# albertz/ParseOggVorbis

Measured on AMD Instinct MI355X. Metric: audio packets/sec (blocksize 2048, stereo), higher is better.
Workload: dtype f32; 1 GPU; config3: 65536 stereo packets, blocksize 2048, 64 streams x 1024, floor+coupling+IMDCT+window+overlap-add; packets_per_gpu=65536, parallelism=streams sharded over 1 GPU(s), no data-path collective

## Files before the change

### parseoggvorbis_amd/csrc/vorbis_synth_hip.hip

```cpp
#include <hip/hip_runtime.h>

#include <mutex>
#include <string>

#include <stdlib.h>

#include "vsyn_host.h"
#include "vsyn_device.h"
#include "vsyn_staged.h"
#include "vsyn_prep.h"
#include "vsyn_fused.h"
#include "vsyn_fused_u.h"
#include "vsyn_vq.h"
#include "vsyn_pcm.h"
#include "vsyn_features.h"
#include "vsyn_spectral.h"
#include "vsyn_spectral_lin.h"
#include "vsyn_chroma.h"
#include "vsyn_spectral_post.h"
#include "vsyn_pcen.h"
#include "vsyn_hpss.h"
#include "vsyn_istft.h"
#include "vsyn_effects.h"
#include "vsyn_pv.h"
// ... 664 lines not shown
  }
  if (!force_staged) {
    FusedArgs a;
    a.cb = h->d_const;
    a.binseg = h->fused.d_binseg;
    a.lds_image = h->fused.d_lds;
    a.packets = d_packets;
    a.segs = d_segments;
    a.info = info;
    a.sinfo = sinfo;
    a.run_cls = h->ws_runcls[wb].p;
    a.runs_per_seg = runs_per_seg;
    a.residue = d_residue;
    a.curve = taps ? taps->floor_curve : nullptr;
    a.fy = fy;
    a.pcm = d_pcm;
    a.carry = h->d_carry;
    a.status = h->d_status;
    a.plane_stride = plane_stride;
    a.S = S;
    a.R = R;
    a.fused_ok = use_u ? (fmask & 1u) : fmask;
    a.coupling_mode = (uint32_t)h->fused.coupling_mode;
    if (staged_may_work) HIPCHK(hipEventRecord(h->ev_join, h->side));
    const bool time_u = use_u && (h->profile_which == 2 || !(fmask & 1u));
    hipError_t e = hipSuccess;
    if (a.fused_ok) {
      if (!time_u && (h->profile_which == 1 || h->profile_which == 2)) HIPCHK(profile_begin(h, s, a.curve ? "vsyn_fused_tap_kernel" : fused_kernel_name(H)));
      e = fused_launch(H, h->fused, a, s);
      if (e != hipSuccess) return fail(err, VSYN_ERR_HIP, "fused launch failed: %s", hipGetErrorString(e));
      if (!time_u && (h->profile_which == 1 || h->profile_which == 2)) HIPCHK(profile_end(h, s));
    }
    if (use_u) {
      FusedArgs au = a;
      au.fused_ok = fmask;
      if (time_u && (h->profile_which == 1 || h->profile_which == 2)) HIPCHK(profile_begin(h, s, au.curve ? "vsyn_fused_u_tap_kernel" : "vsyn_fused_u_kernel"));
      e = u_launch(H, h->utab, au, s);
      if (e != hipSuccess) return fail(err, VSYN_ERR_HIP, "generic fused launch failed: %s", hipGetErrorString(e));
      if (time_u && (h->profile_which == 1 || h->profile_which == 2)) HIPCHK(profile_end(h, s));
    }
    if (staged_may_work) HIPCHK(hipStreamWaitEvent(s, h->ev_join, 0));
  }

  h->last_ran_layout = !prep_kernel;
  h->last_prep_on_main = ps == s;
  h->pre_done_valid[wb] = ps != s;
// ... 1990 lines not shown
```

### parseoggvorbis_amd/csrc/vsyn_fused.h

```cpp
#pragma once
#include <hip/hip_runtime.h>

#include "vsyn_device.h"

#ifndef FUSED_WAVES
#define FUSED_WAVES 16
#endif
#ifndef FUSED_MIN_WAVES_PER_SIMD
#define FUSED_MIN_WAVES_PER_SIMD 4
#endif
#define FUSED_XSLOTS 576
#ifndef VSYN_KNOCKOUT
#define VSYN_KNOCKOUT 0
#endif
#ifdef VSYN_STAMPS
#define VSYN_NSTAMPS 16
__device__ unsigned long long g_vsyn_stamps[8192][VSYN_NSTAMPS];
#define STAMP(i)                                                  \
  do {                                                            \
    __builtin_amdgcn_sched_barrier(0);                            \
    const unsigned long long t_ = __builtin_readcyclecounter();   \
    st_acc[i] += t_ - st_last;                                    \
    st_last = t_;                                                 \
    __builtin_amdgcn_sched_barrier(0);                            \
  } while (0)
#else
#define STAMP(i) do { } while (0)
#endif

struct FusedLdsImage {
  float2 pre[8][64];
  float2 post[8][64];
  float2 tw1[8][64];
  float2 tw2[8][8];
  float win[2][2][8][64];
  float invdb[260];
  float2 pre_s[64];
  float2 post_s[64];
  float2 tws[6][64];
  float wsl[2][64];
  float2 post8[8][8];
  float wsl8[2][8][8];
};

struct FusedTables {
  uint8_t* d_binseg = nullptr;
  FusedLdsImage* d_lds = nullptr;
  int waves_per_cu = 12;
  int coupling_mode = 0;
};

struct FusedArgs {
  const uint8_t* cb;
  const uint8_t* binseg;
  const FusedLdsImage* lds_image;
  const vsyn_packet* packets;
  const vsyn_segment* segs;
  const PktInfo* info;
  const SegInfo* sinfo;
  uint16_t* curve;
  const uint8_t* run_cls;
  const float* residue;
  const uint16_t* fy;
  float* pcm;
  float* carry;
  DevStatus* status;
  uint64_t plane_stride;
  uint32_t S, R, fused_ok, coupling_mode, runs_per_seg;
};

__device__ __forceinline__ float2 f2(float x, float y) { return make_float2(x, y); }
__device__ __forceinline__ float2 cadd(float2 a, float2 b) { return f2(a.x + b.x, a.y + b.y); }
__device__ __forceinline__ float2 csub(float2 a, float2 b) { return f2(a.x - b.x, a.y - b.y); }
__device__ __forceinline__ float2 cmulf(float2 a, float2 b) {
  return f2(__builtin_fmaf(a.x, b.x, -(a.y * b.y)), __builtin_fmaf(a.x, b.y, a.y * b.x));
}
__device__ __forceinline__ float2 mul_mi(float2 a) { return f2(a.y, -a.x); }

__device__ __forceinline__ void dft8(float2 (&x)[8]) {
  const float h = 0.70710678118654752440f;
  float2 a0 = cadd(x[0], x[4]), a1 = cadd(x[1], x[5]), a2 = cadd(x[2], x[6]), a3 = cadd(x[3], x[7]);
  float2 b0 = csub(x[0], x[4]), b1 = csub(x[1], x[5]), b2 = csub(x[2], x[6]), b3 = csub(x[3], x[7]);
  b1 = f2((b1.x + b1.y) * h, (b1.y - b1.x) * h);
  b2 = mul_mi(b2);
  b3 = f2((b3.y - b3.x) * h, -(b3.x + b3.y) * h);
  float2 c0 = cadd(a0, a2), c1 = csub(a0, a2), c2 = cadd(a1, a3), c3 = mul_mi(csub(a1, a3));
  x[0] = cadd(c0, c2);
  x[4] = csub(c0, c2);
  x[2] = cadd(c1, c3);
  x[6] = csub(c1, c3);
  float2 d0 = cadd(b0, b2), d1 = csub(b0, b2), d2 = cadd(b1, b3), d3 = mul_mi(csub(b1, b3));
// ... 98 lines not shown
  k.bad = (r[7] >> 8) & 0xFFu;
  return k;
}
__device__ __forceinline__ PktScalars pkt_load(const PktInfo* p) {
  typedef const __attribute__((address_space(4))) u32x8* const_words;
  return pkt_fields(*(const_words)(uintptr_t)p);
}

enum { K_REG = 0, K_LDS = 1, K_CARRY = 2 };
__device__ __forceinline__ uint32_t bitrev6(uint32_t l) { return __brev(l) >> 26; }

template <int ROLE, bool TAPC>
__device__ __forceinline__ uint32_t fused_short_pass(const FusedArgs& A, const FusedLdsImage& T, float2* __restrict__ xb, const float2* __restrict__ pxb,
                                                     float2* seg2, lds_f32* cbuf, lds_u32* my_flags, const lds_u32* partner_flags, const uint32_t lane,
                                                     const vsyn_segment sg, const SegInfo si, const uint32_t q, const uint32_t qa, const uint32_t qb,
                                                     const uint32_t C, const uint32_t c, float* plane, const PktInfo* ip, const uint32_t epoch,
                                                     const uint32_t prev_kind, const uint32_t prev_half, float (&P)[8], const uint32_t bseg0,
                                                     const uint32_t sidx, const uint32_t xsl, const uint32_t posts, const uint32_t ys_stride, bool& hand_over_out
#ifdef VSYN_STAMPS
                                                     , unsigned long long (&st_acc)[VSYN_NSTAMPS], unsigned long long& st_last
#endif
                                                     ) {
  constexpr uint32_t MS = 128u, ML = 1024u;
  const ConstHeader* H = hdr_of(A.cb);
  typedef uint32_t u32x4 __attribute__((ext_vector_type(4)));
  const uint32_t idx = min(q + (lane & 7u), qb - 1u);
  const u32x4 da = ((const u32x4*)(ip + idx))[0], db = ((const u32x4*)(ip + idx))[1];
  const uint32_t map0 = __builtin_amdgcn_readfirstlane(db[3] & 0xFFu);
  const bool cand = lane < 8u && q + lane < qb;
  const uint64_t okm = __ballot(cand && !((db[3] >> 8) & 0xFFu) && !((db[2] >> 16) & 0xFFu) && (db[3] & 0xFFu) == map0);
  const uint32_t Jp = (uint32_t)__builtin_ctzll(~okm);
  STAMP(9);
  const uint32_t qn = q + Jp, p0 = sg.first_packet + q;
  const uint32_t emit_l = q + (lane & 7u) < qa ? 0u : da[3];
  float2 raw[8];
  uint32_t vrow[8];
#pragma unroll
  for (uint32_t t = 0; t < 8; ++t) {
    const uint32_t tc = min(t, Jp - 1u);
    const uint64_t off = ((uint64_t)__builtin_amdgcn_readlane(da[1], tc) << 32) | (uint32_t)__builtin_amdgcn_readlane(da[0], tc);
    raw[t] = (VSYN_KNOCKOUT & 256) ? f2(0.001f * (float)lane, 0.002f) : ((const float2*)(A.residue + off + (size_t)c * MS))[lane];
    vrow[t] = (A.fy + ((size_t)(p0 + tc) * C + c) * ys_stride)[sidx];
  }
#pragma unroll
  for (uint32_t t = 0; t < 8; ++t)
    if (t >= Jp) raw[t] = f2(0.f, 0.f);
  float2 r[8];
// ... 171 lines not shown
        float* up = out + shift + 2u * kap;
        float* dn = out + shift + MS - 2u - 2u * kap;
#pragma unroll
        for (int j = 0; j < 4; ++j) {
          *(float2*)(up + 16 * j) = f2(oh_s[j], n_s[j]);
          *(float2*)(dn - 16 * j) = f2(n_m[j], oh_m[j]);
        }
      }
    } else if (emit) {
#pragma unroll
      for (int j = 0; j < 4; ++j) {
        const uint32_t s = 2u * kap + 16u * j;
        const uint32_t f0 = s + shift, f1 = s + 1u + shift, f2m = MS - 2u - s + shift, f3m = MS - 1u - s + shift;
        if (f0 < emit) out[f0] = oh_s[j];
        if (f1 < emit) out[f1] = n_s[j];
        if (f2m < emit) out[f2m] = n_m[j];
        if (f3m < emit) out[f3m] = oh_m[j];
      }
    }
  }
  (void)next_emit;
  (void)next_out;
  if ((last_of_segment || hand_over) && jo == Jp - 1u) {
    const size_t carry_half = (size_t)H->max_streams * C * ML;
    float* cout = A.carry + (si.parity_in ^ 1u) * carry_half + ((size_t)sg.stream * C + c) * ML;
#pragma unroll
    for (int k = 0; k < 8; ++k) {
      const uint32_t f = kap + 8u * k;
      const uint32_t s = k >= 4 ? 2u * f - 64u : 63u - 2u * f, sm = MS - 1u - s;
      const float v_s = Pn[k] * wl1[k], v_m = Pn[k] * wl0[k];
      if (last_of_segment) {
        cout[s] = v_s;
        cout[sm] = v_m;
      } else {
        cbuf[s] = v_s;
        cbuf[sm] = v_m;
      }
    }
  }
  {
    const int from = (int)((Jp - 1u) * 8u + kap);
#pragma unroll
    for (int k = 0; k < 8; ++k) P[k] = __shfl(Pn[k], from);
  }
  if (__any(floor_bad)) {
    if (floor_bad) raise_status(A.status, VSYN_ST_FLOOR_VALUE, floor_bad_pkt);
    vmem_drain();
  }
  hand_over_out = hand_over;
  return Jp;
}


template <int ROLE, bool MIXED, bool TAPC, bool RING = false>
__device__ __forceinline__ void fused_run(const FusedArgs& A, const FusedLdsImage& T, float2* __restrict__ xb, const float2* __restrict__ pxb, float4* __restrict__ seg,
                                          lds_f32* cbuf, lds_u32* my_flags, const lds_u32* partner_flags, const uint32_t lane0, const uint32_t g,
                                          const vsyn_segment sg, const SegInfo si, const uint32_t qa, const uint32_t qb, const uint32_t C, const uint32_t c,
                                          const RingLds& rl = RingLds()) {
  static_assert(!(RING && MIXED), "ring mode is a steady-run mode");
  constexpr uint32_t STEP = RING ? 8u : 1u;
  constexpr uint32_t ML = 1024;
  const uint8_t* __restrict__ cb = A.cb;
  const ConstHeader* H = hdr_of(cb);
  const uint32_t num = sg.num_packets;

  float P[8];
#pragma unroll
  for (int k = 0; k < 8; ++k) P[k] = 0.f;
  uint32_t prev_next_long = 1;
  uint32_t prev_kind = K_REG;
  uint32_t prev_half = 0;
  float* const plane = A.pcm + ((size_t)g * C + c) * A.plane_stride;
  const float* cin = nullptr;

  const uint32_t seg_base = (uint32_t)(uintptr_t)(lds_u32*)seg;
  uint32_t bseg[8];
#pragma unroll
  for (int t = 0; t < 8; ++t) bseg[t] = seg_base | (seg_base << 16);
  uint32_t sidx = 0, xsl = 0;
  int cur_floor = -1;
  uint32_t vrow = 0;
  bool vrow_ok = false;

  const uint32_t ys_stride = __builtin_amdgcn_readfirstlane(H->ys_stride);
  const MapConst* const maps = (const MapConst*)(cb + H->off_map);
  const FloorConst* const floors = (const FloorConst*)(cb + H->off_floor);
  uint32_t cur_map = 0xFFFFFFFFu, map_floor = 0, posts = 0;

  const uint32_t q0 = RING ? ((rl.slot == 7u && qa) ? qa - 1u : qa + rl.slot) : (qa ? qa - 1 : 0);
  if (RING && q0 >= qb) return;
  bool ring_dead = false;
  const PktInfo* const ip = A.info + __builtin_amdgcn_readfirstlane(sg.first_packet);
  PktScalars pi = pkt_load(ip + q0);
  float2 raw[8];
  bool raw_ahead = false;
  bool dma_ahead = false;
  uint32_t dma_younger = 0;
  auto issue_dma = [&](uint64_t off, const uint32_t ln) {
    const char* gsrc = (const char*)(A.residue + off) + 16u * ln;
#pragma unroll
    for (int i = 0; i < 4; ++i)
      __builtin_amdgcn_global_load_lds((const __attribute__((address_space(1))) void*)(gsrc + 1024 * i),
                                       (__attribute__((address_space(3))) void*)((lds_u32*)xb + 256 * i), 16, 0, 0);
  };
  if (!MIXED) {
    const float2* src = (const float2*)(A.residue + pi.res_off + (size_t)c * ML) + lane0;
#pragma unroll
    for (int t = 0; t < 8; ++t) raw[t] = stream_load2(src + 64 * t);
  }
  if (MIXED && qa == 0 && si.has_carry && !pi.bad) {
    const size_t carry_half = (size_t)H->max_streams * C * ML;
    cin = A.carry + si.parity_in * carry_half + ((size_t)sg.stream * C + c) * ML;
    const bool carry_long = si.carry_n == 2u * ML;
    prev_half = si.carry_n / 2u;
    if (carry_long && pi.lng) {
      prev_kind = K_CARRY;
    } else {
      const uint32_t base = carry_long ? 448u : 0u;
      if (carry_long)
        for (uint32_t i = lane0; i < min(448u, pi.emit); i += 64) plane[pi.out_pos + i] = cin[i];
      cbuf[lane0] = cin[base + lane0];
      cbuf[lane0 + 64u] = cin[base + lane0 + 64u];
      prev_kind = K_LDS;
    }
  }
  uint32_t lane_v = lane0;
  vmem_drain();
#ifdef VSYN_STAMPS
  unsigned long long st_acc[VSYN_NSTAMPS] = {0, 0, 0, 0, 0, 0, 0, 0, 0, 0, 0, 0, 0, 0, 0, 0};
  unsigned long long st_last = __builtin_readcyclecounter();
#endif
  uint32_t q = q0;
  for (uint32_t it = 0; q < qb; ++it, q += STEP) {
    STAMP(0);
    asm volatile("" : "+v"(lane_v));
    const uint32_t lane = lane_v;
    const uint32_t kappa = ((lane & 7u) << 3) | (lane >> 3);
    const uint32_t p = sg.first_packet + q;
    const bool halo = q < qa, has_next = q + STEP < qb;
    const PktScalars pin = pkt_load(ip + (has_next ? q + STEP : q));
    if (RING) prev_next_long = q ? (pkt_load(ip + q - 1u).widx >> 1) & 1u : 1u;
    const bool lng = !MIXED || pi.lng != 0u;
    const bool nlng = !MIXED || pin.lng != 0u;
    const uint32_t M = lng ? ML : 128u;
    if (MIXED && pi.bad) {
#pragma unroll
      for (int k = 0; k < 8; ++k) P[k] = 0.f;
      prev_kind = K_REG;
      prev_half = 0;
      vrow_ok = false;
      pi = pin;
      continue;
    }
    if (pi.mapping != cur_map) {
      cur_map = pi.mapping;
      {
        typedef const __attribute__((address_space(4))) uint32_t* kptr;
        const uint32_t w = *(kptr)(uintptr_t)((const uint8_t*)maps[cur_map].chfloor + (c & ~3u));
        map_floor = (w >> (8u * (c & 3u))) & 0xFFu;
      }
    }
    if (MIXED && !lng) {
      if (cur_floor != (int)map_floor) {
        const FloorConst* fc = floors + map_floor;
        posts = __builtin_amdgcn_readfirstlane(fc->posts);
        const uint8_t* bs = A.binseg + (size_t)map_floor * ML;
        const uint32_t seg_base0 = (uint32_t)(uintptr_t)(lds_u32*)seg;
#pragma unroll
        for (int t = 0; t < 8; ++t) {
          const uint32_t two = *(const uint16_t*)(bs + 2u * (lane + 64u * t));
          bseg[t] = (seg_base0 + 8u * (two & 0xFFu)) | ((seg_base0 + 8u * (two >> 8)) << 16);
        }
        const bool in = lane < posts;
        sidx = in ? fc->sorted_idx[lane] : 0u;
        xsl = in ? fc->xs_sorted[lane] : 0u;
        cur_floor = (int)map_floor;
        vmem_drain();
      }
      bool ho = false;
      const uint32_t Jp = fused_short_pass<ROLE, TAPC>(A, T, xb, pxb, (float2*)seg, cbuf, my_flags, partner_flags, lane, sg, si, q, qa, qb, C, c, plane, ip, it + 1u,
                                                 prev_kind, prev_half, P, bseg[0], sidx, xsl, posts, ys_stride, ho
#ifdef VSYN_STAMPS
                                                 , st_acc, st_last
#endif
                                                 );
      prev_kind = ho ? K_LDS : K_REG;
      prev_half = 128u;
      prev_next_long = 0u;
      vrow_ok = false;
      q += Jp - 1u;
      pi = pkt_load(ip + min(q + 1u, qb - 1u));
      STAMP(8);
      continue;
    }

    float2 r[8];
    auto residue_rows = [&](const bool L) {
      if (MIXED && L) {
        if (!dma_ahead) {
          issue_dma(pi.res_off + (uint64_t)c * ML, lane);
          dma_younger = 0;
        }
        if (dma_younger == 8u) __builtin_amdgcn_s_waitcnt(0x0F78);
        else vmem_drain();
        dma_ahead = false;
        if (ROLE != 0) {
          pair_post(&my_flags[0], it + 1);
          pair_wait(&partner_flags[0], it + 1);
        }
#pragma unroll
        for (int t = 0; t < 8; ++t) {
          const float2 own = xb[t * 64 + lane];
          if (ROLE == 0) {
            r[t] = own;
          } else {
// ... 30 lines not shown
    };
    if (lng) residue_rows(true);
    else residue_rows(false);
    STAMP(1);
    if (ROLE != 0 && !(VSYN_KNOCKOUT & 1)) pair_post(&my_flags[1], it + 1);
    if (!MIXED) {
      const float2* src = (const float2*)(A.residue + pin.res_off + (size_t)c * ML) + lane;
#pragma unroll
      for (int t = 0; t < 8; ++t) raw[t] = stream_load2(src + 64 * t);
    }
    __builtin_amdgcn_sched_barrier(0);

    bool floor_bad = false;
    float2* const seg2 = (float2*)seg;
    if (VSYN_KNOCKOUT & 16) {
      if (it == 0) seg2[lane] = f2(0.f, 200.5f);
    } else if (!((pi.own >> c) & 1u)) {
      seg2[lane] = f2(0.f, ((pi.used >> c) & 1u) ? 256.5f : 255.5f);
    } else {
      const uint32_t f = map_floor;
      const uint16_t* row = A.fy + ((size_t)p * C + c) * ys_stride;
      uint32_t v = vrow;
      if (cur_floor != (int)f) {
        const FloorConst* fc = floors + f;
        posts = __builtin_amdgcn_readfirstlane(fc->posts);
        const uint8_t* bs = A.binseg + (size_t)f * ML;
#pragma unroll
        for (int t = 0; t < 8; ++t) {
          const uint32_t two = *(const uint16_t*)(bs + 2u * (lane + 64u * t));
          bseg[t] = (seg_base + 8u * (two & 0xFFu)) | ((seg_base + 8u * (two >> 8)) << 16);
        }
        const bool in = lane < posts;
        sidx = in ? fc->sorted_idx[lane] : 0u;
        xsl = in ? fc->xs_sorted[lane] : 0u;
        cur_floor = (int)f;
        v = row[sidx];
        vmem_drain();
      } else if (!vrow_ok) {
        v = row[sidx];
        vmem_drain();
      }
      if (lane >= posts) v = 0;
      const uint64_t mask = __ballot((v >> 15) != 0) | 1ull;
      const uint64_t below = mask & ((2ull << lane) - 1ull);
      const uint32_t lo = 63u - (uint32_t)__clzll((long long)below);
      const uint64_t above = lane < 63u ? (mask >> (lane + 1u)) : 0ull;
      const bool has_hi = above != 0ull;
      const uint32_t hi = lane + (uint32_t)__ffsll((long long)above);
      const uint32_t packed = (xsl << 16) | (v & 0x7FFFu);
      const uint32_t plo = (uint32_t)__shfl((int)packed, (int)lo);
      const uint32_t phi = (uint32_t)__shfl((int)packed, (int)(has_hi ? hi : lo));
      floor_bad = (v & 0x7FFFu) > 255u;
      const float x0 = (float)(plo >> 16), y0 = fminf((float)(plo & 0xFFFFu), 255.f);
      const float x1 = (float)(phi >> 16), y1 = fminf((float)(phi & 0xFFFFu), 255.f);
      const float inv = has_hi ? __builtin_amdgcn_rcpf(x1 - x0) : 0.f;
      const float ady = fabsf(y1 - y0);
      const float a = ady * inv, b = __builtin_fmaf(-ady, x0, 0.5f) * inv;
      seg2[lane] = y1 >= y0 ? f2(a, b + y0) : f2(-a, (y0 + 1.f) - b);
// ... 160 lines not shown
#pragma unroll
        for (int j = 0; j < 4; ++j) {
          if (!MIXED) {
            stream_store2(up + 128 * j, oh_s[j], n_s[j]);
            stream_store2(dn - 128 * j, n_m[j], oh_m[j]);
          } else {
            *(float2*)(up + 128 * j) = f2(oh_s[j], n_s[j]);
            *(float2*)(dn - 128 * j) = f2(n_m[j], oh_m[j]);
          }
        }
      } else if (emit) {
        if (MIXED) dma_younger = 0xFFu;
#pragma unroll
        for (int j = 0; j < 4; ++j) {
          const uint32_t s = 2u * kappa + 128u * j;
          const uint32_t f0 = s + shift, f1 = s + 1u + shift, f2m = 1022u - s + shift, f3m = 1023u - s + shift;
          if (f0 < emit) out[f0] = oh_s[j];
          if (f1 < emit) out[f1] = n_s[j];
          if (f2m < emit) out[f2m] = n_m[j];
          if (f3m < emit) out[f3m] = oh_m[j];
        }
      }
      STAMP(8);
      if (MIXED && (last_of_segment || hand_over)) dma_younger = 0xFFu;
      if (last_of_segment || hand_over) {
        const size_t carry_half = (size_t)H->max_streams * C * ML;
        float* cout = A.carry + (si.parity_in ^ 1u) * carry_half + ((size_t)sg.stream * C + c) * ML;
        float* nxt = plane + pin.out_pos;
        const float (*TN)[8][64] = T.win[cur_next_long];
#pragma unroll
        for (int k = 0; k < 8; ++k) {
          const uint32_t m = kappa + 64u * k;
          const uint32_t s = k >= 4 ? 2u * m - 512u : 511u - 2u * m;
          const float v_s = P[k] * TN[1][k][lane], v_m = P[k] * TN[0][k][lane];
          if (last_of_segment) {
            cout[s] = v_s;
            cout[1023u - s] = v_m;
          } else {
            const uint32_t sm = 1023u - s;
            if (s < 448u) {
              if (s < pin.emit) nxt[s] = v_s;
            } else if (s < 576u) {
              cbuf[s - 448u] = v_s;
            }
            if (sm < 448u) {
              if (sm < pin.emit) nxt[sm] = v_m;
            } else if (sm < 576u) {
              cbuf[sm - 448u] = v_m;
            }
          }
        }
        if (!MIXED) vmem_drain();
      }
    } else {
    }
    if (MIXED) {
      prev_kind = hand_over ? K_LDS : K_REG;
      prev_half = M;
    }
    if (__any(floor_bad)) {
      if (lane == 0) raise_status(A.status, VSYN_ST_FLOOR_VALUE, p);
      vmem_drain();
    }
    prev_next_long = cur_next_long;
    pi = pin;
  }
#ifdef VSYN_STAMPS
  if (lane0 == 0) {
    const uint32_t unit = blockIdx.x * FUSED_WAVES + (threadIdx.x >> 6);
    if (unit < 8192)
      for (int i = 0; i < VSYN_NSTAMPS; ++i) g_vsyn_stamps[unit][i] = i == VSYN_NSTAMPS - 1 ? (unsigned long long)(qb - q0) : st_acc[i];
  }
#endif
}

static_assert(FUSED_WAVES % 2 == 0, "the two channel waves of a run must share a workgroup");
template <bool TAPC>
__device__ __forceinline__ void fused_kernel_body(const FusedArgs& A) {
  struct Lds {
    float4 seg[FUSED_WAVES][64];
    uint32_t flag[FUSED_WAVES][4];
    FusedLdsImage t;
    float2 x[FUSED_WAVES][FUSED_XSLOTS];
    float ring[FUSED_WAVES][8 * 64];
  };
  __shared__ Lds s_lds;
  FusedLdsImage& s_t = s_lds.t;
  float2 (&s_x)[FUSED_WAVES][FUSED_XSLOTS] = s_lds.x;
  float4 (&s_seg)[FUSED_WAVES][64] = s_lds.seg;
  uint32_t (&s_flag)[FUSED_WAVES][4] = s_lds.flag;
  static_assert(sizeof(s_lds.seg) + sizeof(s_lds.flag) < 65536, "floor entry addresses are packed into 16 bits");
  const ConstHeader* H = hdr_of(A.cb);
  const uint32_t wave = __builtin_amdgcn_readfirstlane(threadIdx.x >> 6);
  const uint32_t lane = threadIdx.x & 63u;
  const uint32_t C = H->channels;
  const uint32_t per_seg = A.runs_per_seg * C;
  const uint32_t unit = blockIdx.x * FUSED_WAVES + wave;
  const uint32_t g = __builtin_amdgcn_readfirstlane(unit / per_seg);
  const uint32_t rem = unit - g * per_seg;
  const uint32_t run = __builtin_amdgcn_readfirstlane(rem / C), c = __builtin_amdgcn_readfirstlane(rem % C);
  vsyn_segment sg = {};
  SegInfo si = {};
  uint32_t cls = 0xFFu;
  bool seg_ok = false;
  if (g < A.S) {
    sg = A.segs[g];
    if (sg.stream < H->max_streams && !(sg.residue_off & 3)) {
      seg_ok = true;
      si = A.sinfo[g];
      cls = __builtin_amdgcn_readfirstlane((uint32_t)A.run_cls[(size_t)g * A.runs_per_seg + run]);
    }
  }
  const uint32_t qa = run * A.R;
  const uint32_t qb = min(sg.num_packets, qa + A.R);
  const bool active = (cls == 1u && (A.fused_ok & 1u)) || (cls == 2u && (A.fused_ok & 2u));
  if (!__syncthreads_or(active ? 1 : 0)) return;
  {
    const uint4* src = (const uint4*)A.lds_image;
    uint4* dst = (uint4*)&s_t;
    for (uint32_t i = threadIdx.x; i < sizeof(FusedLdsImage) / 16; i += FUSED_WAVES * 64) dst[i] = src[i];
    if (threadIdx.x < FUSED_WAVES * 4) (&s_flag[0][0])[threadIdx.x] = 0u;
  }
  static_assert(FUSED_WAVES == 16, "ring mode: 8 slots x 2 channels");
  const uint32_t unit0 = blockIdx.x * FUSED_WAVES;
  const bool one_seg = unit0 / per_seg == (unit0 + FUSED_WAVES - 1u) / per_seg;
  const bool ring_ok = C == 2u && one_seg && g < A.S && (A.fused_ok & 1u) && seg_ok && (cls == 1u || qa >= sg.num_packets);
  const bool ring = __syncthreads_and(ring_ok ? 1 : 0);
  if (!ring && !active) return;
  const uint32_t mag = A.coupling_mode == 1 ? 0u : 1u;
  const int role = (A.coupling_mode == 0 || C < 2) ? 0 : (c == mag ? 1 : 2);
  const uint32_t pw = role ? (wave ^ 1u) : wave;
  lds_u32* mf = (lds_u32*)s_flag[wave];
  const lds_u32* pf = (const lds_u32*)s_flag[pw];
  lds_f32* cbw = (lds_f32*)((float*)s_seg[wave] + 128);
  if (ring) {
    const uint32_t slot = wave >> 1, pred = ((slot + 7u) & 7u) * 2u + c, succ = ((slot + 1u) & 7u) * 2u + c;
    RingLds rl;
    rl.mine = (lds_f32*)s_lds.ring[wave];
    rl.pred = (const lds_f32*)s_lds.ring[pred];
    rl.flags = (lds_u32*)&s_flag[wave][2];
    rl.pred_flags = (const lds_u32*)&s_flag[pred][2];
    rl.succ_flags = (const lds_u32*)&s_flag[succ][2];
    rl.slot = slot;
    const uint32_t ca = qa - slot * A.R, ce = min(sg.num_packets, ca + 8u * A.R);
    if (role == 0) fused_run<0, false, TAPC, true>(A, s_t, s_x[wave], s_x[pw], s_seg[wave], cbw, mf, pf, lane, g, sg, si, ca, ce, C, c, rl);
    else if (role == 1) fused_run<1, false, TAPC, true>(A, s_t, s_x[wave], s_x[pw], s_seg[wave], cbw, mf, pf, lane, g, sg, si, ca, ce, C, c, rl);
    else fused_run<2, false, TAPC, true>(A, s_t, s_x[wave], s_x[pw], s_seg[wave], cbw, mf, pf, lane, g, sg, si, ca, ce, C, c, rl);
  } else if (cls == 1u) {
    if (role == 0) fused_run<0, false, TAPC>(A, s_t, s_x[wave], s_x[pw], s_seg[wave], cbw, mf, pf, lane, g, sg, si, qa, qb, C, c);
    else if (role == 1) fused_run<1, false, TAPC>(A, s_t, s_x[wave], s_x[pw], s_seg[wave], cbw, mf, pf, lane, g, sg, si, qa, qb, C, c);
    else fused_run<2, false, TAPC>(A, s_t, s_x[wave], s_x[pw], s_seg[wave], cbw, mf, pf, lane, g, sg, si, qa, qb, C, c);
  } else {
    if (role == 0) fused_run<0, true, TAPC>(A, s_t, s_x[wave], s_x[pw], s_seg[wave], cbw, mf, pf, lane, g, sg, si, qa, qb, C, c);
    else if (role == 1) fused_run<1, true, TAPC>(A, s_t, s_x[wave], s_x[pw], s_seg[wave], cbw, mf, pf, lane, g, sg, si, qa, qb, C, c);
    else fused_run<2, true, TAPC>(A, s_t, s_x[wave], s_x[pw], s_seg[wave], cbw, mf, pf, lane, g, sg, si, qa, qb, C, c);
  }
}

__global__ void __launch_bounds__(FUSED_WAVES * 64, FUSED_MIN_WAVES_PER_SIMD) vsyn_fused_kernel(const FusedArgs A) { fused_kernel_body<false>(A); }
__global__ void __launch_bounds__(FUSED_WAVES * 64, FUSED_MIN_WAVES_PER_SIMD) vsyn_fused_tap_kernel(const FusedArgs A) { fused_kernel_body<true>(A); }

static inline bool fused_supported(const ConstHeader& H) {
  return H.bs[1] == 2048 && H.bs[0] <= 2048 && H.channels <= 2;
}

static inline int fused_coupling_mode(const ConstHeader& H, const uint8_t* host_const) {
  const MapConst* mp = (const MapConst*)(host_const + H.off_map);
  int mode = -2;
  for (uint32_t k = 0; k < H.num_modes; ++k) {
    if (!H.mode_blockflag[k]) continue;
    const MapConst& m = mp[H.mode_mapping[k]];
    if (m.ncoup > 1) return -1;
    const int cur = m.ncoup == 0 ? 0 : (m.coup[0] == 0 ? 1 : 2);
    if (mode == -2) mode = cur;
    else if (mode != cur) return -1;
  }
  return mode == -2 ? 0 : mode;
}
// ... 38 lines not shown
      same = same && cur == want;
    }
    if (same) mask |= 2;
  }
  return mask;
}

static inline hipError_t fused_tables_create(const ConstHeader& H, const uint8_t* host_const, FusedTables* ft, bool debug) {
  const uint32_t half = H.bs[1] / 2;
  std::vector<uint8_t> tab((size_t)H.num_floors * half);
  const FloorConst* fl = (const FloorConst*)(host_const + H.off_floor);
  for (uint32_t f = 0; f < H.num_floors; ++f) {
    uint32_t s = 0;
    for (uint32_t x = 0; x < half; ++x) {
      while (s + 1 < fl[f].posts && fl[f].xs_sorted[s + 1] <= x) ++s;
      tab[(size_t)f * half + x] = (uint8_t)s;
    }
  }
  hipError_t e = hipMalloc((void**)&ft->d_binseg, tab.size());
  if (e != hipSuccess) return e;
  e = hipMemcpy(ft->d_binseg, tab.data(), tab.size(), hipMemcpyHostToDevice);
  if (e != hipSuccess) return e;
  if (fused_supported(H)) {
    std::vector<FusedLdsImage> imgv(1);
    FusedLdsImage& im = imgv[0];
    memset(&im, 0, sizeof(im));
    const float2* pre = (const float2*)(host_const + H.off_pre[1]);
    const float2* post = (const float2*)(host_const + H.off_post[1]);
    const float2* tw = (const float2*)(host_const + H.off_fft[1]);
    const float* win = (const float*)(host_const + H.off_win[1]);
    for (uint32_t l = 0; l < 64; ++l) {
      const uint32_t kappa = ((l & 7u) << 3) | (l >> 3);
      for (uint32_t k = 0; k < 8; ++k) {
        im.pre[k][l] = pre[l + 64 * k];
        im.post[k][l] = post[kappa + 64 * k];
        im.tw1[k][l] = tw[(l * k) & 511u];
        const uint32_t m = kappa + 64 * k;
        const uint32_t s = k >= 4 ? 2 * m - 512 : 511 - 2 * m;
        for (uint32_t f = 0; f < 2; ++f) {
          im.win[f][0][k][l] = win[(size_t)f * H.bs[1] + s];
          im.win[f][1][k][l] = win[(size_t)f * H.bs[1] + 1023 - s];
        }
      }
    }
    for (uint32_t a = 0; a < 8; ++a)
      for (uint32_t c = 0; c < 8; ++c) im.tw2[a][c] = tw[(8 * c * a) & 511u];
    memcpy(im.invdb, host_const + H.off_invdb, 256 * sizeof(float));
    if (H.bs[0] == 256) {
      const float2* pre0 = (const float2*)(host_const + H.off_pre[0]);
// ... 1 lines not shown
      const float2* tw0 = (const float2*)(host_const + H.off_fft[0]);
      const float* win0 = (const float*)(host_const + H.off_win[0]);
      for (uint32_t l = 0; l < 64; ++l) {
        uint32_t m = 0;
        for (int b = 0; b < 6; ++b) m |= ((l >> b) & 1u) << (5 - b);
        im.pre_s[l] = pre0[l];
        im.post_s[l] = post0[m];
        for (int i = 0; i < 6; ++i) {
          const uint32_t d = 32u >> i;
          im.tws[i][l] = tw0[((l & (d - 1u)) * (32u / d)) & 63u];
        }
        const uint32_t sidx = m >= 32 ? 2 * m - 64 : 63 - 2 * m;
        im.wsl[0][l] = win0[sidx];
        im.wsl[1][l] = win0[127 - sidx];
      }
      for (uint32_t cc = 0; cc < 8; ++cc)
        for (uint32_t a = 0; a < 8; ++a) {
          const uint32_t f = a + 8 * cc, s8 = cc >= 4 ? 2 * f - 64 : 63 - 2 * f;
          im.post8[cc][a] = post0[f];
          im.wsl8[0][cc][a] = win0[s8];
          im.wsl8[1][cc][a] = win0[127 - s8];
        }
    }
    e = hipMalloc((void**)&ft->d_lds, sizeof(FusedLdsImage));
    if (e != hipSuccess) return e;
    e = hipMemcpy(ft->d_lds, &im, sizeof(FusedLdsImage), hipMemcpyHostToDevice);
    if (e != hipSuccess) return e;
  }
  ft->coupling_mode = fused_coupling_mode(H, host_const);
  int blocks = 0;
  if (hipOccupancyMaxActiveBlocksPerMultiprocessor(&blocks, vsyn_fused_kernel, FUSED_WAVES * 64, 0) == hipSuccess && blocks > 0)
    ft->waves_per_cu = blocks * FUSED_WAVES;
  if (debug) fprintf(stderr, "vsyn: fused kernel %d workgroups/CU -> %d waves/CU\n", blocks, ft->waves_per_cu);
  return hipSuccess;
}

static inline void fused_tables_destroy(FusedTables* ft) {
  if (ft->d_binseg) (void)hipFree(ft->d_binseg);
  if (ft->d_lds) (void)hipFree(ft->d_lds);
  ft->d_binseg = nullptr;
  ft->d_lds = nullptr;
}

static inline const char* fused_kernel_name(const ConstHeader&) { return "vsyn_fused_kernel"; }
static inline const char* fused_imdct_kernel_name(uint32_t) { return "vsyn_imdct_wave_kernel"; }

static inline uint32_t fused_pick_run_len(uint32_t run_len, int waves_per_cu, uint32_t S, uint32_t channels, uint32_t max_seg_packets, int num_cus) {
  if (run_len) return run_len;
  const uint64_t slots = (uint64_t)num_cus * (uint64_t)waves_per_cu;
// ... 95 lines not shown
}

static inline void fused_stamps_dump() {
#ifdef VSYN_STAMPS
  static unsigned long long host[8192][VSYN_NSTAMPS];
  if (hipMemcpyFromSymbol(host, HIP_SYMBOL(g_vsyn_stamps), sizeof(host)) == hipSuccess) {
    double sum[VSYN_NSTAMPS] = {0};
    unsigned long long waves = 0, pk = 0;
    for (int u = 0; u < 8192; ++u) {
      if (!host[u][VSYN_NSTAMPS - 1]) continue;
      ++waves;
      pk += host[u][VSYN_NSTAMPS - 1];
      for (int i = 0; i + 1 < VSYN_NSTAMPS; ++i) sum[i] += (double)host[u][i];
    }
    if (pk) {
      static const char* nm[VSYN_NSTAMPS - 1] = {"loop", "residue+handoff+couple", "loads+floor setup", "floor product", "mirror+pre-rot", "partner wait 2",
                                                 "fft512", "post+window+overlap", "stores / short pass: stores", "short: descriptors", "short: rows", "short: couple+floor", "short: fft+window", "-", "-"};
      double tot = 0;
      for (int i = 0; i + 1 < VSYN_NSTAMPS; ++i) tot += sum[i];
      fprintf(stderr, "vsyn stamps: %llu waves, %llu wave-packets, %.0f cycles per wave-packet\n", waves, pk, tot / pk);
      for (int i = 0; i + 1 < VSYN_NSTAMPS; ++i) fprintf(stderr, "  %-26s %8.0f cycles  %5.1f %%\n", nm[i], sum[i] / pk, 100.0 * sum[i] / tot);
    }
  }
#endif
}
```

Baseline: 272.1 million packets/s.

## Stage floor lookup tables in LDS and prefetch table image before activity check

Packs the per-mapping channel-to-floor map and the per-floor bin-segment, sorted-index and x-position tables for up to four floors into the LDS image, so floor switches read LDS instead of scattered global and constant loads. The global reads for the LDS image are issued into registers before the segment lookup and activity barrier, hiding their latency behind that setup. Header fields are passed as kernel arguments, and the first packet's floor row load is hoisted before the loop. It also adds wall-clock start-up instrumentation under the stamps build flag. The cost is more LDS per workgroup and more registers held for the staged copy.

```diff
diff --git a/parseoggvorbis_amd/csrc/vorbis_synth_hip.hip b/parseoggvorbis_amd/csrc/vorbis_synth_hip.hip
--- a/parseoggvorbis_amd/csrc/vorbis_synth_hip.hip
+++ b/parseoggvorbis_amd/csrc/vorbis_synth_hip.hip
@@ -710,6 +710,11 @@
     a.R = R;
     a.fused_ok = use_u ? (fmask & 1u) : fmask;
     a.coupling_mode = (uint32_t)h->fused.coupling_mode;
+    a.channels = H.channels;
+    a.ys_stride = H.ys_stride;
+    a.off_floor = H.off_floor;
+    a.max_streams = H.max_streams;
+    a.lds_floors = h->fused.lds_floors;
     if (staged_may_work) HIPCHK(hipEventRecord(h->ev_join, h->side));
     const bool time_u = use_u && (h->profile_which == 2 || !(fmask & 1u));
     hipError_t e = hipSuccess;
diff --git a/parseoggvorbis_amd/csrc/vsyn_fused.h b/parseoggvorbis_amd/csrc/vsyn_fused.h
--- a/parseoggvorbis_amd/csrc/vsyn_fused.h
+++ b/parseoggvorbis_amd/csrc/vsyn_fused.h
@@ -16,6 +16,11 @@
 #ifdef VSYN_STAMPS
 #define VSYN_NSTAMPS 16
 __device__ unsigned long long g_vsyn_stamps[8192][VSYN_NSTAMPS];
+__device__ unsigned long long g_vsyn_wall[8192][5];
+#define WALL_FIRST_STORE(cond)                                                   \
+  do {                                                                           \
+    if (!wall_store && (cond)) wall_store = (unsigned long long)wall_clock64(); \
+  } while (0)
 #define STAMP(i)                                                  \
   do {                                                            \
     __builtin_amdgcn_sched_barrier(0);                            \
@@ -26,6 +31,7 @@
   } while (0)
 #else
 #define STAMP(i) do { } while (0)
+#define WALL_FIRST_STORE(cond) do { } while (0)
 #endif
 
 struct FusedLdsImage {
@@ -43,9 +49,29 @@
   float wsl8[2][8][8];
 };
 
+#define FUSED_LDS_FLOORS 4
+struct FusedFloorLane {
+  uint32_t iv[4][64];
+  uint32_t sx[64];
+};
+struct FusedFloorImage {
+  uint32_t chfloor[VSYN_MAX_TABLES];
+  uint32_t posts[FUSED_LDS_FLOORS];
+  FusedFloorLane rec[FUSED_LDS_FLOORS];
+};
+struct FusedStagedImage {
+  FusedLdsImage t;
+  FusedFloorImage fl;
+};
+static_assert(sizeof(FusedLdsImage) % 16 == 0 && offsetof(FusedStagedImage, fl) == sizeof(FusedLdsImage) && offsetof(FusedFloorImage, rec) % 16 == 0 &&
+                  sizeof(FusedFloorLane) % 16 == 0,
+              "the staging copy moves whole 16-byte words");
+#define FUSED_STAGE_ROUNDS ((sizeof(FusedStagedImage) / 16 + FUSED_WAVES * 64 - 1) / (FUSED_WAVES * 64))
+
 struct FusedTables {
   uint8_t* d_binseg = nullptr;
   FusedLdsImage* d_lds = nullptr;
+  uint32_t lds_floors = 0;
   int waves_per_cu = 12;
   int coupling_mode = 0;
 };
@@ -67,6 +93,7 @@
   DevStatus* status;
   uint64_t plane_stride;
   uint32_t S, R, fused_ok, coupling_mode, runs_per_seg;
+  uint32_t channels, ys_stride, off_floor, max_streams, lds_floors;
 };
 
 __device__ __forceinline__ float2 f2(float x, float y) { return make_float2(x, y); }
@@ -211,7 +238,6 @@
 #endif
                                                      ) {
   constexpr uint32_t MS = 128u, ML = 1024u;
-  const ConstHeader* H = hdr_of(A.cb);
   typedef uint32_t u32x4 __attribute__((ext_vector_type(4)));
   const uint32_t idx = min(q + (lane & 7u), qb - 1u);
   const u32x4 da = ((const u32x4*)(ip + idx))[0], db = ((const u32x4*)(ip + idx))[1];
@@ -429,7 +455,7 @@
   (void)next_emit;
   (void)next_out;
   if ((last_of_segment || hand_over) && jo == Jp - 1u) {
-    const size_t carry_half = (size_t)H->max_streams * C * ML;
+    const size_t carry_half = (size_t)A.max_streams * C * ML;
     float* cout = A.carry + (si.parity_in ^ 1u) * carry_half + ((size_t)sg.stream * C + c) * ML;
 #pragma unroll
     for (int k = 0; k < 8; ++k) {
@@ -460,7 +486,7 @@
 
 
 template <int ROLE, bool MIXED, bool TAPC, bool RING = false>
-__device__ __forceinline__ void fused_run(const FusedArgs& A, const FusedLdsImage& T, float2* __restrict__ xb, const float2* __restrict__ pxb, float4* __restrict__ seg,
+__device__ __forceinline__ void fused_run(const FusedArgs& A, const FusedLdsImage& T, const FusedFloorImage& FL, float2* __restrict__ xb, const float2* __restrict__ pxb, float4* __restrict__ seg,
                                           lds_f32* cbuf, lds_u32* my_flags, const lds_u32* partner_flags, const uint32_t lane0, const uint32_t g,
                                           const vsyn_segment sg, const SegInfo si, const uint32_t qa, const uint32_t qb, const uint32_t C, const uint32_t c,
                                           const RingLds& rl = RingLds()) {
@@ -468,7 +494,6 @@
   constexpr uint32_t STEP = RING ? 8u : 1u;
   constexpr uint32_t ML = 1024;
   const uint8_t* __restrict__ cb = A.cb;
-  const ConstHeader* H = hdr_of(cb);
   const uint32_t num = sg.num_packets;
 
   float P[8];
@@ -489,10 +514,40 @@
   uint32_t vrow = 0;
   bool vrow_ok = false;
 
-  const uint32_t ys_stride = __builtin_amdgcn_readfirstlane(H->ys_stride);
-  const MapConst* const maps = (const MapConst*)(cb + H->off_map);
-  const FloorConst* const floors = (const FloorConst*)(cb + H->off_floor);
+  const uint32_t ys_stride = A.ys_stride;
+  const FloorConst* const floors = (const FloorConst*)(cb + A.off_floor);
   uint32_t cur_map = 0xFFFFFFFFu, map_floor = 0, posts = 0;
+  auto floor_of_map = [&](const uint32_t m) {
+    return __builtin_amdgcn_readfirstlane((FL.chfloor[min(m, (uint32_t)VSYN_MAX_TABLES - 1u)] >> (8u * (c & 3u))) & 0xFFu);
+  };
+  auto floor_consts = [&](const uint32_t f, const uint32_t ln) {
+    if (f < A.lds_floors) {
+      const FusedFloorLane& fr = FL.rec[f];
+      posts = __builtin_amdgcn_readfirstlane(FL.posts[f]);
+#pragma unroll
+      for (int j = 0; j < 4; ++j) {
+        const uint32_t w = fr.iv[j][ln];
+        bseg[2 * j] = (seg_base + 8u * (w & 0xFFu)) | ((seg_base + 8u * ((w >> 8) & 0xFFu)) << 16);
+        bseg[2 * j + 1] = (seg_base + 8u * ((w >> 16) & 0xFFu)) | ((seg_base + 8u * (w >> 24)) << 16);
+      }
+      const uint32_t sx = fr.sx[ln];
+      sidx = sx & 0xFFFFu;
+      xsl = sx >> 16;
+    } else {
+      const FloorConst* fc = floors + f;
+      posts = __builtin_amdgcn_readfirstlane(fc->posts);
+      const uint8_t* bs = A.binseg + (size_t)f * ML;
+#pragma unroll
+      for (int t = 0; t < 8; ++t) {
+        const uint32_t two = *(const uint16_t*)(bs + 2u * (ln + 64u * t));
+        bseg[t] = (seg_base + 8u * (two & 0xFFu)) | ((seg_base + 8u * (two >> 8)) << 16);
+      }
+      const bool in = ln < posts;
+      sidx = in ? fc->sorted_idx[ln] : 0u;
+      xsl = in ? fc->xs_sorted[ln] : 0u;
+    }
+    cur_floor = (int)f;
+  };
 
   const uint32_t q0 = RING ? ((rl.slot == 7u && qa) ? qa - 1u : qa + rl.slot) : (qa ? qa - 1 : 0);
   if (RING && q0 >= qb) return;
@@ -515,8 +570,18 @@
 #pragma unroll
     for (int t = 0; t < 8; ++t) raw[t] = stream_load2(src + 64 * t);
   }
+  if (!pi.bad && (!MIXED || pi.lng) && pi.mapping < (uint32_t)VSYN_MAX_TABLES && ((pi.own >> c) & 1u)) {
+    const uint32_t f0 = floor_of_map(pi.mapping);
+    if (f0 < A.lds_floors) {
+      cur_map = pi.mapping;
+      map_floor = f0;
+      floor_consts(f0, lane0);
+      vrow = (A.fy + ((size_t)(sg.first_packet + q0) * C + c) * ys_stride)[sidx];
+      vrow_ok = true;
+    }
+  }
   if (MIXED && qa == 0 && si.has_carry && !pi.bad) {
-    const size_t carry_half = (size_t)H->max_streams * C * ML;
+    const size_t carry_half = (size_t)A.max_streams * C * ML;
     cin = A.carry + si.parity_in * carry_half + ((size_t)sg.stream * C + c) * ML;
     const bool carry_long = si.carry_n == 2u * ML;
     prev_half = si.carry_n / 2u;
@@ -536,10 +601,15 @@
 #ifdef VSYN_STAMPS
   unsigned long long st_acc[VSYN_NSTAMPS] = {0, 0, 0, 0, 0, 0, 0, 0, 0, 0, 0, 0, 0, 0, 0, 0};
   unsigned long long st_last = __builtin_readcyclecounter();
+  const unsigned long long wall_loop = (unsigned long long)wall_clock64();
+  unsigned long long wall_store = 0, wall_its = 0;
 #endif
   uint32_t q = q0;
   for (uint32_t it = 0; q < qb; ++it, q += STEP) {
     STAMP(0);
+#ifdef VSYN_STAMPS
+    ++wall_its;
+#endif
     asm volatile("" : "+v"(lane_v));
     const uint32_t lane = lane_v;
     const uint32_t kappa = ((lane & 7u) << 3) | (lane >> 3);
@@ -561,28 +631,12 @@
     }
     if (pi.mapping != cur_map) {
       cur_map = pi.mapping;
-      {
-        typedef const __attribute__((address_space(4))) uint32_t* kptr;
-        const uint32_t w = *(kptr)(uintptr_t)((const uint8_t*)maps[cur_map].chfloor + (c & ~3u));
-        map_floor = (w >> (8u * (c & 3u))) & 0xFFu;
-      }
+      map_floor = floor_of_map(cur_map);
     }
     if (MIXED && !lng) {
       if (cur_floor != (int)map_floor) {
-        const FloorConst* fc = floors + map_floor;
-        posts = __builtin_amdgcn_readfirstlane(fc->posts);
-        const uint8_t* bs = A.binseg + (size_t)map_floor * ML;
-        const uint32_t seg_base0 = (uint32_t)(uintptr_t)(lds_u32*)seg;
-#pragma unroll
-        for (int t = 0; t < 8; ++t) {
-          const uint32_t two = *(const uint16_t*)(bs + 2u * (lane + 64u * t));
-          bseg[t] = (seg_base0 + 8u * (two & 0xFFu)) | ((seg_base0 + 8u * (two >> 8)) << 16);
-        }
-        const bool in = lane < posts;
-        sidx = in ? fc->sorted_idx[lane] : 0u;
-        xsl = in ? fc->xs_sorted[lane] : 0u;
-        cur_floor = (int)map_floor;
-        vmem_drain();
+        floor_consts(map_floor, lane);
+        if (map_floor >= A.lds_floors) vmem_drain();
       }
       bool ho = false;
       const uint32_t Jp = fused_short_pass<ROLE, TAPC>(A, T, xb, pxb, (float2*)seg, cbuf, my_flags, partner_flags, lane, sg, si, q, qa, qb, C, c, plane, ip, it + 1u,
@@ -598,6 +652,7 @@
       q += Jp - 1u;
       pi = pkt_load(ip + min(q + 1u, qb - 1u));
       STAMP(8);
+      WALL_FIRST_STORE(q + 1u > qa);
       continue;
     }
 
@@ -674,18 +729,7 @@
       const uint16_t* row = A.fy + ((size_t)p * C + c) * ys_stride;
       uint32_t v = vrow;
       if (cur_floor != (int)f) {
-        const FloorConst* fc = floors + f;
-        posts = __builtin_amdgcn_readfirstlane(fc->posts);
-        const uint8_t* bs = A.binseg + (size_t)f * ML;
-#pragma unroll
-        for (int t = 0; t < 8; ++t) {
-          const uint32_t two = *(const uint16_t*)(bs + 2u * (lane + 64u * t));
-          bseg[t] = (seg_base + 8u * (two & 0xFFu)) | ((seg_base + 8u * (two >> 8)) << 16);
-        }
-        const bool in = lane < posts;
-        sidx = in ? fc->sorted_idx[lane] : 0u;
-        xsl = in ? fc->xs_sorted[lane] : 0u;
-        cur_floor = (int)f;
+        floor_consts(f, lane);
         v = row[sidx];
         vmem_drain();
       } else if (!vrow_ok) {
@@ -892,9 +936,10 @@
         }
       }
       STAMP(8);
+      WALL_FIRST_STORE(emit != 0u);
       if (MIXED && (last_of_segment || hand_over)) dma_younger = 0xFFu;
       if (last_of_segment || hand_over) {
-        const size_t carry_half = (size_t)H->max_streams * C * ML;
+        const size_t carry_half = (size_t)A.max_streams * C * ML;
         float* cout = A.carry + (si.parity_in ^ 1u) * carry_half + ((size_t)sg.stream * C + c) * ML;
         float* nxt = plane + pin.out_pos;
         const float (*TN)[8][64] = T.win[cur_next_long];
@@ -940,6 +985,12 @@
     const uint32_t unit = blockIdx.x * FUSED_WAVES + (threadIdx.x >> 6);
     if (unit < 8192)
       for (int i = 0; i < VSYN_NSTAMPS; ++i) g_vsyn_stamps[unit][i] = i == VSYN_NSTAMPS - 1 ? (unsigned long long)(qb - q0) : st_acc[i];
+    if (unit < 8192) {
+      g_vsyn_wall[unit][1] = wall_loop;
+      g_vsyn_wall[unit][2] = wall_store;
+      g_vsyn_wall[unit][3] = (unsigned long long)wall_clock64();
+      g_vsyn_wall[unit][4] = wall_its;
+    }
   }
 #endif
 }
@@ -950,20 +1001,35 @@
   struct Lds {
     float4 seg[FUSED_WAVES][64];
     uint32_t flag[FUSED_WAVES][4];
-    FusedLdsImage t;
+    FusedStagedImage t;
     float2 x[FUSED_WAVES][FUSED_XSLOTS];
     float ring[FUSED_WAVES][8 * 64];
   };
   __shared__ Lds s_lds;
-  FusedLdsImage& s_t = s_lds.t;
+  static_assert(sizeof(Lds) <= 160 * 1024, "one workgroup's LDS");
+  FusedStagedImage& s_t = s_lds.t;
   float2 (&s_x)[FUSED_WAVES][FUSED_XSLOTS] = s_lds.x;
   float4 (&s_seg)[FUSED_WAVES][64] = s_lds.seg;
   uint32_t (&s_flag)[FUSED_WAVES][4] = s_lds.flag;
   static_assert(sizeof(s_lds.seg) + sizeof(s_lds.flag) < 65536, "floor entry addresses are packed into 16 bits");
-  const ConstHeader* H = hdr_of(A.cb);
   const uint32_t wave = __builtin_amdgcn_readfirstlane(threadIdx.x >> 6);
   const uint32_t lane = threadIdx.x & 63u;
-  const uint32_t C = H->channels;
+#ifdef VSYN_STAMPS
+  if (lane == 0 && blockIdx.x * FUSED_WAVES + wave < 8192) {
+    unsigned long long* w = g_vsyn_wall[blockIdx.x * FUSED_WAVES + wave];
+    w[0] = (unsigned long long)wall_clock64();
+    w[1] = w[2] = w[3] = w[4] = 0;
+  }
+#endif
+  const uint32_t stage_words = (uint32_t)((sizeof(FusedLdsImage) + offsetof(FusedFloorImage, rec)) / 16) + A.lds_floors * (uint32_t)(sizeof(FusedFloorLane) / 16);
+  uint4 stage[FUSED_STAGE_ROUNDS];
+#pragma unroll
+  for (uint32_t k = 0; k < FUSED_STAGE_ROUNDS; ++k) {
+    const uint32_t i = threadIdx.x + k * FUSED_WAVES * 64;
+    stage[k] = make_uint4(0u, 0u, 0u, 0u);
+    if (i < stage_words) stage[k] = ((const uint4*)A.lds_image)[i];
+  }
+  const uint32_t C = A.channels;
   const uint32_t per_seg = A.runs_per_seg * C;
   const uint32_t unit = blockIdx.x * FUSED_WAVES + wave;
   const uint32_t g = __builtin_amdgcn_readfirstlane(unit / per_seg);
@@ -975,7 +1041,7 @@
   bool seg_ok = false;
   if (g < A.S) {
     sg = A.segs[g];
-    if (sg.stream < H->max_streams && !(sg.residue_off & 3)) {
+    if (sg.stream < A.max_streams && !(sg.residue_off & 3)) {
       seg_ok = true;
       si = A.sinfo[g];
       cls = __builtin_amdgcn_readfirstlane((uint32_t)A.run_cls[(size_t)g * A.runs_per_seg + run]);
@@ -986,9 +1052,12 @@
   const bool active = (cls == 1u && (A.fused_ok & 1u)) || (cls == 2u && (A.fused_ok & 2u));
   if (!__syncthreads_or(active ? 1 : 0)) return;
   {
-    const uint4* src = (const uint4*)A.lds_image;
     uint4* dst = (uint4*)&s_t;
-    for (uint32_t i = threadIdx.x; i < sizeof(FusedLdsImage) / 16; i += FUSED_WAVES * 64) dst[i] = src[i];
+#pragma unroll
+    for (uint32_t k = 0; k < FUSED_STAGE_ROUNDS; ++k) {
+      const uint32_t i = threadIdx.x + k * FUSED_WAVES * 64;
+      if (i < stage_words) dst[i] = stage[k];
+    }
     if (threadIdx.x < FUSED_WAVES * 4) (&s_flag[0][0])[threadIdx.x] = 0u;
   }
   static_assert(FUSED_WAVES == 16, "ring mode: 8 slots x 2 channels");
@@ -1013,17 +1082,17 @@
     rl.succ_flags = (const lds_u32*)&s_flag[succ][2];
     rl.slot = slot;
     const uint32_t ca = qa - slot * A.R, ce = min(sg.num_packets, ca + 8u * A.R);
-    if (role == 0) fused_run<0, false, TAPC, true>(A, s_t, s_x[wave], s_x[pw], s_seg[wave], cbw, mf, pf, lane, g, sg, si, ca, ce, C, c, rl);
-    else if (role == 1) fused_run<1, false, TAPC, true>(A, s_t, s_x[wave], s_x[pw], s_seg[wave], cbw, mf, pf, lane, g, sg, si, ca, ce, C, c, rl);
-    else fused_run<2, false, TAPC, true>(A, s_t, s_x[wave], s_x[pw], s_seg[wave], cbw, mf, pf, lane, g, sg, si, ca, ce, C, c, rl);
+    if (role == 0) fused_run<0, false, TAPC, true>(A, s_t.t, s_t.fl, s_x[wave], s_x[pw], s_seg[wave], cbw, mf, pf, lane, g, sg, si, ca, ce, C, c, rl);
+    else if (role == 1) fused_run<1, false, TAPC, true>(A, s_t.t, s_t.fl, s_x[wave], s_x[pw], s_seg[wave], cbw, mf, pf, lane, g, sg, si, ca, ce, C, c, rl);
+    else fused_run<2, false, TAPC, true>(A, s_t.t, s_t.fl, s_x[wave], s_x[pw], s_seg[wave], cbw, mf, pf, lane, g, sg, si, ca, ce, C, c, rl);
   } else if (cls == 1u) {
-    if (role == 0) fused_run<0, false, TAPC>(A, s_t, s_x[wave], s_x[pw], s_seg[wave], cbw, mf, pf, lane, g, sg, si, qa, qb, C, c);
-    else if (role == 1) fused_run<1, false, TAPC>(A, s_t, s_x[wave], s_x[pw], s_seg[wave], cbw, mf, pf, lane, g, sg, si, qa, qb, C, c);
-    else fused_run<2, false, TAPC>(A, s_t, s_x[wave], s_x[pw], s_seg[wave], cbw, mf, pf, lane, g, sg, si, qa, qb, C, c);
+    if (role == 0) fused_run<0, false, TAPC>(A, s_t.t, s_t.fl, s_x[wave], s_x[pw], s_seg[wave], cbw, mf, pf, lane, g, sg, si, qa, qb, C, c);
+    else if (role == 1) fused_run<1, false, TAPC>(A, s_t.t, s_t.fl, s_x[wave], s_x[pw], s_seg[wave], cbw, mf, pf, lane, g, sg, si, qa, qb, C, c);
+    else fused_run<2, false, TAPC>(A, s_t.t, s_t.fl, s_x[wave], s_x[pw], s_seg[wave], cbw, mf, pf, lane, g, sg, si, qa, qb, C, c);
   } else {
-    if (role == 0) fused_run<0, true, TAPC>(A, s_t, s_x[wave], s_x[pw], s_seg[wave], cbw, mf, pf, lane, g, sg, si, qa, qb, C, c);
-    else if (role == 1) fused_run<1, true, TAPC>(A, s_t, s_x[wave], s_x[pw], s_seg[wave], cbw, mf, pf, lane, g, sg, si, qa, qb, C, c);
-    else fused_run<2, true, TAPC>(A, s_t, s_x[wave], s_x[pw], s_seg[wave], cbw, mf, pf, lane, g, sg, si, qa, qb, C, c);
+    if (role == 0) fused_run<0, true, TAPC>(A, s_t.t, s_t.fl, s_x[wave], s_x[pw], s_seg[wave], cbw, mf, pf, lane, g, sg, si, qa, qb, C, c);
+    else if (role == 1) fused_run<1, true, TAPC>(A, s_t.t, s_t.fl, s_x[wave], s_x[pw], s_seg[wave], cbw, mf, pf, lane, g, sg, si, qa, qb, C, c);
+    else fused_run<2, true, TAPC>(A, s_t.t, s_t.fl, s_x[wave], s_x[pw], s_seg[wave], cbw, mf, pf, lane, g, sg, si, qa, qb, C, c);
   }
 }
 
@@ -1108,9 +1177,26 @@
   e = hipMemcpy(ft->d_binseg, tab.data(), tab.size(), hipMemcpyHostToDevice);
   if (e != hipSuccess) return e;
   if (fused_supported(H)) {
-    std::vector<FusedLdsImage> imgv(1);
-    FusedLdsImage& im = imgv[0];
-    memset(&im, 0, sizeof(im));
+    std::vector<FusedStagedImage> imgv(1);
+    memset(&imgv[0], 0, sizeof(FusedStagedImage));
+    FusedLdsImage& im = imgv[0].t;
+    {
+      FusedFloorImage& fi = imgv[0].fl;
+      const MapConst* mp = (const MapConst*)(host_const + H.off_map);
+      for (uint32_t m = 0; m < H.num_mappings && m < VSYN_MAX_TABLES; ++m)
+        for (uint32_t ch = 0; ch < 4 && ch < VSYN_MAX_CHANNELS; ++ch) fi.chfloor[m] |= (uint32_t)mp[m].chfloor[ch] << (8u * ch);
+      ft->lds_floors = std::min<uint32_t>(H.num_floors, FUSED_LDS_FLOORS);
+      for (uint32_t f = 0; f < ft->lds_floors; ++f) {
+        fi.posts[f] = fl[f].posts;
+        for (uint32_t l = 0; l < 64; ++l) {
+          for (uint32_t t = 0; t < 8; ++t) {
+            const uint8_t* two = &tab[(size_t)f * half + 2u * (l + 64u * t)];
+            fi.rec[f].iv[t >> 1][l] |= ((uint32_t)two[0] | ((uint32_t)two[1] << 8)) << (16u * (t & 1u));
+          }
+          if (l < fl[f].posts) fi.rec[f].sx[l] = (uint32_t)fl[f].sorted_idx[l] | ((uint32_t)fl[f].xs_sorted[l] << 16);
+        }
+      }
+    }
     const float2* pre = (const float2*)(host_const + H.off_pre[1]);
     const float2* post = (const float2*)(host_const + H.off_post[1]);
     const float2* tw = (const float2*)(host_const + H.off_fft[1]);
@@ -1158,9 +1244,9 @@
           im.wsl8[1][cc][a] = win0[127 - s8];
         }
     }
-    e = hipMalloc((void**)&ft->d_lds, sizeof(FusedLdsImage));
+    e = hipMalloc((void**)&ft->d_lds, sizeof(FusedStagedImage));
     if (e != hipSuccess) return e;
-    e = hipMemcpy(ft->d_lds, &im, sizeof(FusedLdsImage), hipMemcpyHostToDevice);
+    e = hipMemcpy(ft->d_lds, &imgv[0], sizeof(FusedStagedImage), hipMemcpyHostToDevice);
     if (e != hipSuccess) return e;
   }
   ft->coupling_mode = fused_coupling_mode(H, host_const);
@@ -1302,5 +1388,35 @@
       for (int i = 0; i + 1 < VSYN_NSTAMPS; ++i) fprintf(stderr, "  %-26s %8.0f cycles  %5.1f %%\n", nm[i], sum[i] / pk, 100.0 * sum[i] / tot);
     }
   }
+  static unsigned long long wall[8192][5];
+  if (hipMemcpyFromSymbol(wall, HIP_SYMBOL(g_vsyn_wall), sizeof(wall)) == hipSuccess) {
+    unsigned long long t0 = ~0ull, t1 = 0;
+    std::vector<double> v[5];
+    for (int u = 0; u < 8192; ++u) {
+      if (!wall[u][0]) continue;
+      t0 = std::min(t0, wall[u][0]);
+      t1 = std::max(t1, wall[u][3]);
+    }
+    for (int u = 0; u < 8192; ++u) {
+      if (!wall[u][0] || !wall[u][2] || !wall[u][4]) continue;
+      v[0].push_back((double)(wall[u][0] - t0) / 100.0);
+      v[1].push_back((double)(wall[u][1] - t0) / 100.0);
+      v[2].push_back((double)(wall[u][2] - t0) / 100.0);
+      v[3].push_back((double)(wall[u][2] - wall[u][0]) / 100.0);
+      v[4].push_back((double)(wall[u][3] - wall[u][1]) / 100.0 / (double)wall[u][4]);
+    }
+    if (!v[0].empty()) {
+      static const char* wn[5] = {"wave entry", "packet loop entry", "first PCM store issued", "entry -> first PCM store", "steady step (loop time / iterations)"};
+      fprintf(stderr, "vsyn start-up: %zu waves with PCM, kernel %.2f us (earliest entry to latest end); us min / median / max\n", v[0].size(),
+              (double)(t1 - t0) / 100.0);
+      double med[5];
+      for (int i = 0; i < 5; ++i) {
+        std::sort(v[i].begin(), v[i].end());
+        med[i] = v[i][v[i].size() / 2];
+        fprintf(stderr, "  %-38s %8.2f %8.2f %8.2f\n", wn[i], v[i].front(), med[i], v[i].back());
+      }
+      fprintf(stderr, "  recoverable: median (entry -> first PCM store) - median steady step = %.2f us\n", med[3] - med[4]);
+    }
+  }
 #endif
 }
```

Result: no change. 274.6 million packets/s, median of 5 (+0.9%).
